# 0xEigenLabs/eigen-zkvm

Hardware: AMD Instinct MI355X
Metric: Goldilocks NTT GElems/s + BN254 G1 MSM Mpts/s; starky prove ms at 2^24 rows (higher is better)
Workload: dtype u64 (Goldilocks, canonical)

## Files before the change

### eigen-zkvm_amd/csrc/ntt.hip

```cpp
#include "zk_internal.h"
#include "ntt_reg.hip.h"
#include <map>
#include <mutex>
#include <type_traits>
#include <vector>

namespace zk {

namespace {

constexpr int NTT_TILE = 4096;
constexpr int TW_LO_BITS = 12;
constexpr int TW_LO = 1 << TW_LO_BITS;

struct PassParams {
    const u64* in;
    u64* out;
    const u64* w256;
    const u64* tw_lo;
    const u64* tw_hi;
    const u64* tw_mid;
    u64 pre_scale;
    u32 dshift;
    const u64* sc_lo;
    const u64* sc_hi;
    u64 sc_cinv;
    u64 out_scale;
    u64 inner;
    u64 valid_in;
    u64 s_np;
    u32 np;
    u32 log_s;
    u32 has_tw;
};

__device__ __forceinline__ u64 tab2(const u64* __restrict__ lo, const u64* __restrict__ hi, u64 e) {
    return gl::mul_tw_nc(hi[e >> TW_LO_BITS], lo[e & (TW_LO - 1)]);
}

template <int LOGA, int LOGB, bool KMODE, bool INV>
__global__ __launch_bounds__(NTT_TILE / 16) void ntt_pass_kernel(const PassParams P) {
    constexpr int LOGR = LOGA + LOGB, R = 1 << LOGR, RA = 1 << LOGA, RB = 1 << LOGB;
    constexpr int C = NTT_TILE / R;
    constexpr int GA = 16 / RA, GB = 16 / RB;
    constexpr int TG = R / 16;
    constexpr int PAD = KMODE ? 512 / R : 0;
    constexpr int ROW = RB * C + PAD;
    static_assert(LOGR >= 4 && LOGR <= 8 && LOGA <= 4 && LOGB <= 4, "tile shape");
    __shared__ u64 lds[RA * ROW];
    __shared__ u64 sfac[RB * C];

    const int t = threadIdx.x;
    const u64 u0 = (u64)blockIdx.x * C;

    auto split = [&](u64 u, u64& p, u64& rem) {
        const u64 uc = u < P.inner ? u : 0;
        if (P.np == 1) { p = uc >> P.log_s; rem = uc & (((u64)1 << P.log_s) - 1); }
        else if ((P.inner >> 32) == 0) { const u32 p32 = (u32)uc / (u32)P.s_np; p = p32; rem = (u32)uc - p32 * (u32)P.s_np; }
        else
        { p = uc / P.s_np; rem = uc - p * P.s_np; }
    };
    auto row_of = [&](u64 rem) { return P.np == 1 ? rem : (P.inner >> 32) == 0 ? (u64)((u32)rem / P.np) : rem / P.np; };
    const bool small = ((P.inner * R) >> 29) == 0;
    int cB, tb;
    if (KMODE) { tb = t % TG; cB = t / TG; } else { cB = t % C; tb = t / C; }

    const bool split_f = (P.has_tw && !P.tw_mid) || P.sc_lo;
    u64 fa_hi[GB], fa_lo[GB], fs_hi[GA], fs_lo[GA], fa[GB];
#pragma unroll
    for (int g = 0; g < GB; ++g) fa_hi[g] = fa_lo[g] = fa[g] = 1;
#pragma unroll
    for (int m = 0; m < GA; ++m) fs_hi[m] = fs_lo[m] = 1;
    auto issue_factor_loads = [&]() {
        const u64* __restrict__ lo = P.sc_lo ? P.sc_lo : P.tw_lo;
        const u64* __restrict__ hi = P.sc_lo ? P.sc_hi : P.tw_hi;
        u64 p, rem;
        split(u0 + cB, p, rem);
        const u32 rq = P.sc_lo ? (u32)row_of(rem) : 0;
#pragma unroll
        for (int g = 0; g < GB; ++g) {
            const u32 ka = tb + g * TG;
            const u32 e = P.sc_lo ? (ka << P.log_s) + rq : ((u32)p * ka) << P.log_s;
            fa_hi[g] = hi[e >> TW_LO_BITS]; fa_lo[g] = lo[e & (TW_LO - 1)];
        }
#pragma unroll
        for (int m = 0; m < GA; ++m) {
            const int i = t + m * (NTT_TILE / 16);
            const u32 kb = i / C;
            split(u0 + i % C, p, rem);
            const u32 e = P.sc_lo ? (RA * kb) << P.log_s : ((u32)p * (RA * kb)) << P.log_s;
            fs_hi[m] = hi[e >> TW_LO_BITS]; fs_lo[m] = lo[e & (TW_LO - 1)];
        }
    };

    {
        const int c = t % C, ta = t / C;
        const u64 u = u0 + c;
        const bool live = u < P.inner;
        u64 x[GA][RA];
        const bool full = u0 + C <= P.inner && (u64)(R - 1) * P.inner + u0 + C <= P.valid_in;
        const u64* __restrict__ base = P.in + (u64)(ta * GA) * P.inner + (live ? u : 0);
        if (full) {
#pragma unroll
            for (int g = 0; g < GA; ++g)
#pragma unroll
                for (int ja = 0; ja < RA; ++ja) x[g][ja] = base[(u64)(ja * RB + g) * P.inner];
        } else {
#pragma unroll
            for (int g = 0; g < GA; ++g)
#pragma unroll
                for (int ja = 0; ja < RA; ++ja) {
                    const u64 off = (u64)(ja * RB + g) * P.inner;
                    const bool ok = live && (u64)(ta * GA) * P.inner + off + u < P.valid_in;
                    const u64 v = *(ok ? base + off : P.in);
                    x[g][ja] = ok ? v : 0;
                }
        }
        if (split_f) issue_factor_loads();
#pragma unroll
        for (int g = 0; g < GA; ++g) ntt_reg<LOGA, INV>(x[g]);
        if (LOGR <= 6 && C >= 64 && LOGB > 0 && P.pre_scale == 1) {
            static_for<0, TG>([&](auto TA) {
                constexpr int ta_c = decltype(TA)::value;
                if (ta == ta_c) {
                    static_for<0, GA>([&](auto GI) {
                        constexpr int g = decltype(GI)::value, jb = ta_c * GA + g;
                        static_for<0, RA>([&](auto KA) {
                            constexpr int ka = decltype(KA)::value;
                            constexpr int e0 = (39 * (64 / (R > 64 ? 64 : R)) * jb * ka) % 192, e = INV ? (192 - e0) % 192 : e0;
                            u64 v = x[g][bitrev_c(ka, LOGA)];
                            if constexpr (e >= 96) v = gl::neg(gl::mul_pow2<e - 96>(v));
                            else v = gl::mul_pow2<e>(v);
                            lds[ka * ROW + jb * C + c] = v;
                        });
                    });
                }
            });
        } else
        {
#pragma unroll
            for (int g = 0; g < GA; ++g) {
                const int jb = ta * GA + g;
#pragma unroll
                for (int ka = 0; ka < RA; ++ka) {
                    u64 v = x[g][bitrev_c(ka, LOGA)];
                    if (LOGB > 0 && ka > 0) v = gl::mul_tw(v, P.w256[(jb * ka) << (8 - LOGR)]);
                    else if (P.pre_scale != 1) v = gl::mul_tw(v, P.pre_scale);
                    lds[ka * ROW + jb * C + c] = v;
                }
            }
        }
    }
    if (split_f) {
#pragma unroll
        for (int m = 0; m < GA; ++m) {
            u64 sv = gl::mul_tw_nc(fs_hi[m], fs_lo[m]);
            if (P.sc_lo) sv = gl::mul_tw_nc(sv, P.sc_cinv);
            sfac[t + m * (NTT_TILE / 16)] = sv;
        }
#pragma unroll
        for (int g = 0; g < GB; ++g) fa[g] = gl::mul_tw_nc(fa_hi[g], fa_lo[g]);
    }
    __syncthreads();
    {
        const int c = cB;
        const u64 u = u0 + c;
        u64 y[GB][RB];
#pragma unroll
        for (int g = 0; g < GB; ++g) {
            const int ka = tb + g * TG;
#pragma unroll
            for (int jb = 0; jb < RB; ++jb) y[g][jb] = lds[ka * ROW + jb * C + c];
        }
        u64 p, rem;
        split(u, p, rem);
        u64 tw[GB][RB];
        if (P.tw_mid) {
            const u32 sh = P.log_s - P.dshift, istep = (((u32)p * RA) << sh) * 8;
#pragma unroll
            for (int g = 0; g < GB; ++g) {
                const u32 ka = tb + g * TG, i0 = (((u32)p * ka) << sh) * 8;
#pragma unroll
                for (int kb = 0; kb < RB; ++kb) tw[g][kb] = *(const u64*)((const char*)P.tw_mid + (u32)(i0 + kb * istep));
            }
        }
#pragma unroll
        for (int g = 0; g < GB; ++g) ntt_reg<LOGB, INV>(y[g]);
        if (u >= P.inner) return;

        auto finish = [&](auto small_c) {
            constexpr bool SMALL = decltype(small_c)::value;
            u64* __restrict__ outp = P.out + p * R * P.s_np + rem;
            const u64 kstride = P.s_np;
            const u32 b0 = ((u32)p * R * (u32)P.s_np + (u32)rem) * 8, bstep = RA * (u32)P.s_np * 8;
            auto put = [&](int g, int kb, u64 v) {
                const u32 ka = tb + g * TG;
                if constexpr (SMALL) *(u64*)((char*)P.out + (u32)(b0 + ka * (u32)P.s_np * 8 + kb * bstep)) = v;
                else outp[(u64)(RA * kb + ka) * kstride] = v;
            };
            if (P.tw_mid) {
#pragma unroll
                for (int g = 0; g < GB; ++g)
#pragma unroll
                    for (int kb = 0; kb < RB; ++kb) put(g, kb, gl::mul_tw(y[g][bitrev_c(kb, LOGB)], tw[g][kb]));
            } else if (split_f) {
#pragma unroll
                for (int g = 0; g < GB; ++g)
#pragma unroll
                    for (int kb = 0; kb < RB; ++kb) {
                        const u64 f = kb == 0 ? fa[g] : gl::mul_tw_nc(fa[g], sfac[kb * C + c]);
                        put(g, kb, gl::mul_tw(y[g][bitrev_c(kb, LOGB)], f));
                    }
            } else if (P.out_scale != 1) {
#pragma unroll
                for (int g = 0; g < GB; ++g)
#pragma unroll
                    for (int kb = 0; kb < RB; ++kb) put(g, kb, gl::mul_tw(y[g][bitrev_c(kb, LOGB)], P.out_scale));
            } else {
#pragma unroll
                for (int g = 0; g < GB; ++g)
#pragma unroll
                    for (int kb = 0; kb < RB; ++kb) put(g, kb, y[g][bitrev_c(kb, LOGB)]);
            }
        };
        if (small) finish(std::true_type{});
        else finish(std::false_type{});
    }
}

__global__ void ntt_small_kernel(const u64* in, u64* out, u32 np, u32 n_in, u32 n, u64 w, u64 g, u64 cst) {
    const u32 tid = blockIdx.x * blockDim.x + threadIdx.x;
    if (tid >= n * np) return;
    const u32 k = tid / np, c = tid % np;
    const u64 wk = gl::pow(w, k);
    u64 acc = 0, cur = 1;
    for (u32 i = 0; i < n_in; ++i) { acc = gl::add(acc, gl::mul(in[(u64)i * np + c], cur)); cur = gl::mul(cur, wk); }
    out[(u64)k * np + c] = gl::mul(acc, gl::mul(cst, gl::pow(g, k)));
}

struct Tables { DevConst w256, w256s, lo, hi, mid; u32 dshift = 0; };
struct ScaleTables { DevConst lo, hi; };

std::mutex g_mu;
auto& g_tables = *new std::map<std::pair<int, std::pair<u32, int>>, Tables>;
auto& g_scales = *new std::map<std::pair<int, std::pair<u32, u64>>, ScaleTables>;

void two_level(u64 base, u64 cst, u32 nbits, std::vector<u64>& lo, std::vector<u64>& hi) {
    lo.resize(TW_LO);
    u64 c = cst;
    for (int i = 0; i < TW_LO; ++i) { lo[i] = c; c = gl::hmul(c, base); }
    size_t nh = nbits > (u32)TW_LO_BITS ? (size_t)1 << (nbits - TW_LO_BITS) : 1;
    hi.resize(nh);
    u64 step = gl::hpow(base, TW_LO);
    c = 1;
    for (size_t i = 0; i < nh; ++i) { hi[i] = c; c = gl::hmul(c, step); }
}

const Tables& get_tables(u32 nbits, bool inverse) {
    int dev; ZK_HIP(hipGetDevice(&dev));
    std::lock_guard<std::mutex> lk(g_mu);
    auto key = std::make_pair(dev, std::make_pair(nbits, (int)inverse));
    auto it = g_tables.find(key);
    if (it != g_tables.end()) return it->second;
    u64 w = gl::hroot(nbits), w8 = gl::hroot(8);
    if (inverse) { w = gl::hinv(w); w8 = gl::hinv(w8); }
    std::vector<u64> t256(256), lo, hi;
    u64 c = 1;
    for (int i = 0; i < 256; ++i) { t256[i] = c; c = gl::hmul(c, w8); }
    two_level(w, 1, nbits, lo, hi);
    Tables T; T.w256 = DevConst(t256); T.lo = DevConst(lo); T.hi = DevConst(hi);
    if (inverse) {
        const u64 ninv = gl::hinv((1ull << nbits) % GL_P);
        std::vector<u64> t256s(256);
        for (int i = 0; i < 256; ++i) t256s[i] = gl::hmul(t256[i], ninv);
        T.w256s = DevConst(t256s);
    }
    {
        T.dshift = nbits > 16 ? nbits - 16 : 0;
        const size_t nm = (size_t)1 << (nbits - T.dshift);
        std::vector<u64> mid(nm);
        const u64 step = gl::hpow(w, 1ull << T.dshift);
        c = 1;
        for (size_t i = 0; i < nm; ++i) { mid[i] = c; c = gl::hmul(c, step); }
        T.mid = DevConst(mid);
    }
    return g_tables.emplace(key, std::move(T)).first->second;
}

const ScaleTables& get_scale(u32 nbits, u64 g, u64 cst) {
    int dev; ZK_HIP(hipGetDevice(&dev));
    std::lock_guard<std::mutex> lk(g_mu);
    auto key = std::make_pair(dev, std::make_pair(nbits, g));
    auto it = g_scales.find(key);
    if (it != g_scales.end()) return it->second;
    std::vector<u64> lo, hi;
    two_level(g, cst, nbits, lo, hi);
    ScaleTables S; S.lo = DevConst(lo); S.hi = DevConst(hi);
    return g_scales.emplace(key, std::move(S)).first->second;
}

template <int LOGA, int LOGB>
void launch_pass(const PassParams& P, bool kmode, bool inverse, hipStream_t st) {
    constexpr int C = NTT_TILE >> (LOGA + LOGB);
    const u64 blocks = (P.inner + C - 1) / C;
    ZK_REQUIRE(blocks < (1ull << 31), "ntt: grid too large");
    const dim3 g((u32)blocks), b(NTT_TILE / 16);
    const int variant = (kmode ? 2 : 0) | (inverse ? 1 : 0);
#define ZK_PASS(K, I) hipLaunchKernelGGL((ntt_pass_kernel<LOGA, LOGB, K, I>), g, b, 0, st, P)
    switch (variant) {
        case 0: ZK_PASS(false, false); break; case 1: ZK_PASS(false, true); break;
        case 2: ZK_PASS(true, false); break;  default: ZK_PASS(true, true); break;
    }
#undef ZK_PASS
    ZK_HIP(hipGetLastError());
}

void launch_pass_logr(int logr, const PassParams& P, bool kmode, bool inverse, hipStream_t st) {
    switch (logr) {
        case 4: launch_pass<2, 2>(P, kmode, inverse, st); break;
        case 5: launch_pass<3, 2>(P, kmode, inverse, st); break;
        case 6: launch_pass<3, 3>(P, kmode, inverse, st); break;
        case 7: launch_pass<4, 3>(P, kmode, inverse, st); break;
        case 8: launch_pass<4, 4>(P, kmode, inverse, st); break;
        default: throw Error("ntt: unsupported pass radix");
    }
}

std::vector<int> plan(u32 nbits) {
    std::vector<int> r;
    if (nbits < 4) return r;
    int np = (nbits + 7) / 8;
    int base = nbits / np, extra = nbits % np;
    for (int i = 0; i < np; ++i) r.push_back(base + (i < extra ? 1 : 0));
    return r;
}

struct Scale { bool on = false; u64 g = 1, cst = 1; };

void run_transform(const u64* in, u64* a, u64* b,
                   u32 n_pols, u32 nbits, u64 valid_rows, bool inverse, Scale sc, u64 out_scale, hipStream_t st) {
    const u64 n = 1ull << nbits;
    if (nbits < 4) {
        u64 w = gl::hroot(nbits);
        if (inverse) w = gl::hinv(w);
        u64 cst = sc.on ? sc.cst : out_scale;
        u64 g = sc.on ? sc.g : 1;
        u32 total = (u32)(n * n_pols);
        hipLaunchKernelGGL(ntt_small_kernel, dim3((total + 255) / 256), dim3(256), 0, st, in, a, n_pols,
                           (u32)valid_rows, (u32)n, w, g, cst);
        ZK_HIP(hipGetLastError());
        return;
    }
    const std::vector<int> radices = plan(nbits);
    const int np = (int)radices.size();
    const Tables& T = get_tables(nbits, inverse);
    const ScaleTables* S = sc.on ? &get_scale(nbits, sc.g, sc.cst) : nullptr;
    u32 log_s = 0;
    const u64* cur = in;
    for (int i = 0; i < np; ++i) {
        const int logr = radices[i];
        u64* dstbuf = ((np - 1 - i) % 2 == 0) ? a : b;
        const bool last = (i == np - 1);
        PassParams P{};
        P.in = cur; P.out = dstbuf;
        P.w256 = T.w256.u(); P.tw_lo = T.lo.u(); P.tw_hi = T.hi.u();
        P.sc_lo = (last && sc.on) ? S->lo.u() : nullptr;
        P.sc_hi = (last && sc.on) ? S->hi.u() : nullptr;
        P.sc_cinv = (last && sc.on) ? gl::hinv(sc.cst) : 1;
        P.out_scale = 1; P.pre_scale = 1;
        if (last && !sc.on && out_scale != 1) {
            ZK_REQUIRE(inverse && out_scale == gl::hinv(n % GL_P), "ntt: unsupported constant scaling");
            P.w256 = T.w256s.u(); P.pre_scale = out_scale;
        }
        P.inner = (n >> logr) * n_pols;
        P.valid_in = (i == 0) ? valid_rows * n_pols : n * n_pols;
        P.s_np = ((u64)1 << log_s) * n_pols;
        P.np = n_pols;
        P.log_s = log_s;
        P.has_tw = last ? 0 : 1;
        P.dshift = T.dshift;
        P.tw_mid = (!last && log_s >= T.dshift) ? T.mid.u() : nullptr;
        const bool kmode = P.s_np < 16;
        launch_pass_logr(logr, P, kmode, inverse, st);
        cur = dstbuf;
        log_s += logr;
    }
}

}

int ntt_num_passes(uint32_t nbits) { return nbits < 4 ? 1 : (int)plan(nbits).size(); }

const u64* ntt_w256_table(bool inverse) { return get_tables(8, inverse).w256.u(); }

void ntt_dev(const u64* d_src, u64* d_dst, u64* d_tmp, uint32_t n_pols, uint32_t nbits, bool inverse, hipStream_t st) {
    ZK_REQUIRE(nbits <= 32, "ntt: nbits > 32");
    if (n_pols == 0) return;
    ZK_REQUIRE(d_src != d_dst, "ntt: dst may not alias src");
    u64 out_scale = inverse ? gl::hinv((1ull << nbits) % GL_P) : 1;
    run_transform(d_src, d_dst, d_tmp, n_pols, nbits, 1ull << nbits, inverse, Scale{}, out_scale, st);
}

void lde_dev(const u64* d_src, u64* d_dst, u64* d_tmp, uint32_t n_pols, uint32_t nbits, uint32_t nbits_ext, hipStream_t st) {
    ZK_REQUIRE(nbits_ext <= 32 && nbits <= nbits_ext, "lde: need nbits <= nbits_ext <= 32");
    if (n_pols == 0) return;
    ZK_REQUIRE(d_src != d_dst, "lde: dst may not alias src");
    const u64 n = 1ull << nbits;
    Scale sc; sc.on = true; sc.g = 49; sc.cst = gl::hinv(n % GL_P);
    const int fwd_passes = ntt_num_passes(nbits_ext);
    u64* first_fwd_out = ((fwd_passes - 1) % 2 == 0) ? d_dst : d_tmp;
    u64* coef = (first_fwd_out == d_dst) ? d_tmp : d_dst;
    u64* other = (coef == d_dst) ? d_tmp : d_dst;
    run_transform(d_src, coef, other, n_pols, nbits, n, true, sc, 1, st);
    run_transform(coef, d_dst, d_tmp, n_pols, nbits_ext, n, false, Scale{}, 1, st);
}

}
```

Before: 79.01.

## Replace LDS factor tables with per-thread recurrence twiddles and nontemporal input loads

Drops the shared-memory factor staging (sfac) and early factor-table loads. Each thread now does one table lookup per output group and steps the twiddle or coset factor by repeated multiplication with a per-pass constant step computed on the host. Input loads are also marked nontemporal. This saves table gathers, LDS traffic and registers, at the cost of a serial chain of extra multiplies per group and table loads that no longer overlap the global reads.

Result: faster. 86.70 (median of 6 runs) (+9.7%).

```diff
diff --git a/eigen-zkvm_amd/csrc/ntt.hip b/eigen-zkvm_amd/csrc/ntt.hip
--- a/eigen-zkvm_amd/csrc/ntt.hip
+++ b/eigen-zkvm_amd/csrc/ntt.hip
@@ -24,7 +24,7 @@
     u32 dshift;
     const u64* sc_lo;
     const u64* sc_hi;
-    u64 sc_cinv;
+    u64 sc_step;
     u64 out_scale;
     u64 inner;
     u64 valid_in;
@@ -48,50 +48,9 @@
     constexpr int ROW = RB * C + PAD;
     static_assert(LOGR >= 4 && LOGR <= 8 && LOGA <= 4 && LOGB <= 4, "tile shape");
     __shared__ u64 lds[RA * ROW];
-    __shared__ u64 sfac[RB * C];
 
     const int t = threadIdx.x;
     const u64 u0 = (u64)blockIdx.x * C;
-
-    auto split = [&](u64 u, u64& p, u64& rem) {
-        const u64 uc = u < P.inner ? u : 0;
-        if (P.np == 1) { p = uc >> P.log_s; rem = uc & (((u64)1 << P.log_s) - 1); }
-        else if ((P.inner >> 32) == 0) { const u32 p32 = (u32)uc / (u32)P.s_np; p = p32; rem = (u32)uc - p32 * (u32)P.s_np; }
-        else
-        { p = uc / P.s_np; rem = uc - p * P.s_np; }
-    };
-    auto row_of = [&](u64 rem) { return P.np == 1 ? rem : (P.inner >> 32) == 0 ? (u64)((u32)rem / P.np) : rem / P.np; };
-    const bool small = ((P.inner * R) >> 29) == 0;
-    int cB, tb;
-    if (KMODE) { tb = t % TG; cB = t / TG; } else { cB = t % C; tb = t / C; }
-
-    const bool split_f = (P.has_tw && !P.tw_mid) || P.sc_lo;
-    u64 fa_hi[GB], fa_lo[GB], fs_hi[GA], fs_lo[GA], fa[GB];
-#pragma unroll
-    for (int g = 0; g < GB; ++g) fa_hi[g] = fa_lo[g] = fa[g] = 1;
-#pragma unroll
-    for (int m = 0; m < GA; ++m) fs_hi[m] = fs_lo[m] = 1;
-    auto issue_factor_loads = [&]() {
-        const u64* __restrict__ lo = P.sc_lo ? P.sc_lo : P.tw_lo;
-        const u64* __restrict__ hi = P.sc_lo ? P.sc_hi : P.tw_hi;
-        u64 p, rem;
-        split(u0 + cB, p, rem);
-        const u32 rq = P.sc_lo ? (u32)row_of(rem) : 0;
-#pragma unroll
-        for (int g = 0; g < GB; ++g) {
-            const u32 ka = tb + g * TG;
-            const u32 e = P.sc_lo ? (ka << P.log_s) + rq : ((u32)p * ka) << P.log_s;
-            fa_hi[g] = hi[e >> TW_LO_BITS]; fa_lo[g] = lo[e & (TW_LO - 1)];
-        }
-#pragma unroll
-        for (int m = 0; m < GA; ++m) {
-            const int i = t + m * (NTT_TILE / 16);
-            const u32 kb = i / C;
-            split(u0 + i % C, p, rem);
-            const u32 e = P.sc_lo ? (RA * kb) << P.log_s : ((u32)p * (RA * kb)) << P.log_s;
-            fs_hi[m] = hi[e >> TW_LO_BITS]; fs_lo[m] = lo[e & (TW_LO - 1)];
-        }
-    };
 
     {
         const int c = t % C, ta = t / C;
@@ -104,7 +63,7 @@
 #pragma unroll
             for (int g = 0; g < GA; ++g)
 #pragma unroll
-                for (int ja = 0; ja < RA; ++ja) x[g][ja] = base[(u64)(ja * RB + g) * P.inner];
+                for (int ja = 0; ja < RA; ++ja) x[g][ja] = __builtin_nontemporal_load(&base[(u64)(ja * RB + g) * P.inner]);
         } else {
 #pragma unroll
             for (int g = 0; g < GA; ++g)
@@ -112,11 +71,10 @@
                 for (int ja = 0; ja < RA; ++ja) {
                     const u64 off = (u64)(ja * RB + g) * P.inner;
                     const bool ok = live && (u64)(ta * GA) * P.inner + off + u < P.valid_in;
-                    const u64 v = *(ok ? base + off : P.in);
+                    const u64 v = __builtin_nontemporal_load(ok ? base + off : P.in);
                     x[g][ja] = ok ? v : 0;
                 }
         }
-        if (split_f) issue_factor_loads();
 #pragma unroll
         for (int g = 0; g < GA; ++g) ntt_reg<LOGA, INV>(x[g]);
         if (LOGR <= 6 && C >= 64 && LOGB > 0 && P.pre_scale == 1) {
@@ -151,19 +109,10 @@
             }
         }
     }
-    if (split_f) {
-#pragma unroll
-        for (int m = 0; m < GA; ++m) {
-            u64 sv = gl::mul_tw_nc(fs_hi[m], fs_lo[m]);
-            if (P.sc_lo) sv = gl::mul_tw_nc(sv, P.sc_cinv);
-            sfac[t + m * (NTT_TILE / 16)] = sv;
-        }
-#pragma unroll
-        for (int g = 0; g < GB; ++g) fa[g] = gl::mul_tw_nc(fa_hi[g], fa_lo[g]);
-    }
     __syncthreads();
     {
-        const int c = cB;
+        int c, tb;
+        if (KMODE) { tb = t % TG; c = t / TG; } else { c = t % C; tb = t / C; }
         const u64 u = u0 + c;
         u64 y[GB][RB];
 #pragma unroll
@@ -172,8 +121,12 @@
 #pragma unroll
             for (int jb = 0; jb < RB; ++jb) y[g][jb] = lds[ka * ROW + jb * C + c];
         }
+        const u64 uc = u < P.inner ? u : 0;
         u64 p, rem;
-        split(u, p, rem);
+        if (P.np == 1) { p = uc >> P.log_s; rem = uc & (((u64)1 << P.log_s) - 1); }
+        else if ((P.inner >> 32) == 0) { const u32 p32 = (u32)uc / (u32)P.s_np; p = p32; rem = (u32)uc - p32 * (u32)P.s_np; }
+        else
+        { p = uc / P.s_np; rem = uc - p * P.s_np; }
         u64 tw[GB][RB];
         if (P.tw_mid) {
             const u32 sh = P.log_s - P.dshift, istep = (((u32)p * RA) << sh) * 8;
@@ -193,37 +146,46 @@
             u64* __restrict__ outp = P.out + p * R * P.s_np + rem;
             const u64 kstride = P.s_np;
             const u32 b0 = ((u32)p * R * (u32)P.s_np + (u32)rem) * 8, bstep = RA * (u32)P.s_np * 8;
-            auto put = [&](int g, int kb, u64 v) {
-                const u32 ka = tb + g * TG;
+            auto put = [&](u32 ka, int kb, u64 v) {
                 if constexpr (SMALL) *(u64*)((char*)P.out + (u32)(b0 + ka * (u32)P.s_np * 8 + kb * bstep)) = v;
                 else outp[(u64)(RA * kb + ka) * kstride] = v;
             };
+            const u64 row_q = !P.sc_lo ? 0 : P.np == 1 ? rem : (P.inner >> 32) == 0 ? (u64)((u32)rem / P.np) : rem / P.np;
             if (P.tw_mid) {
 #pragma unroll
-                for (int g = 0; g < GB; ++g)
-#pragma unroll
-                    for (int kb = 0; kb < RB; ++kb) put(g, kb, gl::mul_tw(y[g][bitrev_c(kb, LOGB)], tw[g][kb]));
-            } else if (split_f) {
-#pragma unroll
-                for (int g = 0; g < GB; ++g)
+                for (int g = 0; g < GB; ++g) {
+                    const int ka = tb + g * TG;
 #pragma unroll
                     for (int kb = 0; kb < RB; ++kb) {
-                        const u64 f = kb == 0 ? fa[g] : gl::mul_tw_nc(fa[g], sfac[kb * C + c]);
-                        put(g, kb, gl::mul_tw(y[g][bitrev_c(kb, LOGB)], f));
+                        u64 v = y[g][bitrev_c(kb, LOGB)];
+                        v = gl::mul_tw(v, tw[g][kb]);
+                        put(ka, kb, v);
                     }
-            } else if (P.out_scale != 1) {
-#pragma unroll
-                for (int g = 0; g < GB; ++g)
-#pragma unroll
-                    for (int kb = 0; kb < RB; ++kb) put(g, kb, gl::mul_tw(y[g][bitrev_c(kb, LOGB)], P.out_scale));
-            } else {
-#pragma unroll
-                for (int g = 0; g < GB; ++g)
-#pragma unroll
-                    for (int kb = 0; kb < RB; ++kb) put(g, kb, y[g][bitrev_c(kb, LOGB)]);
+                }
+                return;
+            }
+            u64 tw_step = 1;
+            if (P.has_tw) tw_step = tab2(P.tw_lo, P.tw_hi, (p * RA) << P.log_s);
+#pragma unroll
+            for (int g = 0; g < GB; ++g) {
+                const int ka = tb + g * TG;
+                u64 f = P.out_scale;
+                if (P.has_tw) f = tab2(P.tw_lo, P.tw_hi, (p * ka) << P.log_s);
+                if (P.sc_lo) f = tab2(P.sc_lo, P.sc_hi, ((u64)ka << P.log_s) + row_q);
+                const bool scaled = P.has_tw || P.sc_lo || P.out_scale != 1;
+                const u64 fstep = P.sc_lo ? P.sc_step : tw_step;
+#pragma unroll
+                for (int kb = 0; kb < RB; ++kb) {
+                    u64 v = y[g][bitrev_c(kb, LOGB)];
+                    if (scaled) {
+                        v = gl::mul_tw(v, f);
+                        if (kb + 1 < RB) f = gl::mul_tw_nc(f, fstep);
+                    }
+                    put(ka, kb, v);
+                }
             }
         };
-        if (small) finish(std::true_type{});
+        if (((P.inner * R) >> 29) == 0) finish(std::true_type{});
         else finish(std::false_type{});
     }
 }
@@ -366,7 +328,8 @@
         P.w256 = T.w256.u(); P.tw_lo = T.lo.u(); P.tw_hi = T.hi.u();
         P.sc_lo = (last && sc.on) ? S->lo.u() : nullptr;
         P.sc_hi = (last && sc.on) ? S->hi.u() : nullptr;
-        P.sc_cinv = (last && sc.on) ? gl::hinv(sc.cst) : 1;
+        const int loga = (logr + 1) / 2;
+        P.sc_step = (last && sc.on) ? gl::hpow(sc.g, (1ull << loga) << log_s) : 1;
         P.out_scale = 1; P.pre_scale = 1;
         if (last && !sc.on && out_scale != 1) {
             ZK_REQUIRE(inverse && out_scale == gl::hinv(n % GL_P), "ntt: unsupported constant scaling");
```
